# JaehaKim97/EDTR

Hardware: AMD Instinct MI355X
Metric: restored 512x512 images/sec @ 4 denoise steps (higher is better)
Workload: dtype bf16; 1 GPU; EDTR-det s4 (sd21): vae_encode + q_sample(t=200) + 4 x (ControlNet+UNet) + vae_decode, batch 8/GPU of 512x512; global_batch=8, image_size=512, denoise_steps=4, parallelism=batch-sharded x1, graphs=True, batches_in_flight=2, precision=fast

## Files before the change

edtr_amd/csrc/norm.hip:

```cpp
#include <stdlib.h>
#include "common.h"

namespace {

template <typename T>
struct IO16 {
    using in_t = uint16_t;
    using out_t = uint16_t;
    static __device__ __forceinline__ void load8(const in_t* p, float (&f)[8]) { unpack8<T>(ldg16(p), f); }
    static __device__ __forceinline__ void store8(out_t* p, int, const float (&f)[8]) { stg16(p, pack8<T>(f)); }
};
template <typename OT, int PARTS>
struct IOF32 {
    using in_t = float;
    using out_t = uint16_t;
    static __device__ __forceinline__ void load8(const in_t* p, float (&f)[8]) {
        const f32x4 a = *reinterpret_cast<const f32x4*>(p), b = *reinterpret_cast<const f32x4*>(p + 4);
#pragma unroll
        for (int j = 0; j < 4; ++j) { f[j] = a[j]; f[j + 4] = b[j]; }
    }
    static __device__ __forceinline__ void store8(out_t* p, int C, const float (&f)[8]) {
        const U4 hi = pack8<OT>(f);
        stg16(p, hi);
        if constexpr (PARTS >= 2) {
            float lo[8], back[8];
            unpack8<OT>(hi, back);
#pragma unroll
            for (int j = 0; j < 8; ++j) lo[j] = f[j] - back[j];
            stg16(p + C, pack8<OT>(lo));
        }
        if constexpr (PARTS == 3) stg16(p + 2 * C, hi);
    }
};
using IOF32S = IOF32<BF16, 3>;

template <typename F>
bool with_io(int dtype, F&& body) {
    switch (dtype) {
        case EDTR_BF16: body(IO16<BF16>{}); return true;
        case EDTR_F16: body(IO16<F16>{}); return true;
        case EDTR_F32_SPLIT: body(IOF32<BF16, 3>{}); return true;
        case EDTR_F32_H1: body(IOF32<F16, 1>{}); return true;
        case EDTR_F32_H2: body(IOF32<F16, 2>{}); return true;
        case EDTR_F32_H3: body(IOF32<F16, 3>{}); return true;
        default: return false;
    }
}

template <typename IO>
__global__ void gn_stats_kernel(const edtr_gn_params p, int CV, int R, int ppb) {
    using in_t = typename IO::in_t;
    extern __shared__ __attribute__((aligned(16))) char smem_raw[];
    float* red = reinterpret_cast<float*>(smem_raw);
    const int tid = threadIdx.x;
    const int b = blockIdx.y;
    const int C = p.C;
    const int cpg = C / p.groups;
    const int64_t pix0 = (int64_t)blockIdx.x * ppb;
    const int npix = (int)min((int64_t)ppb, (int64_t)p.HW - pix0);
    const in_t* xb = static_cast<const in_t*>(p.x) + ((int64_t)b * p.HW + pix0) * p.ldx;
    const int nslots = (CV + blockDim.x - 1) / blockDim.x;
    for (int slot = 0; slot < nslots; ++slot) {
        const int cv = R > 1 ? tid % CV : tid + slot * (int)blockDim.x;
        const int r = R > 1 ? tid / CV : 0;
        if (cv >= CV || r >= R) continue;
        float s[8], q[8];
#pragma unroll
        for (int j = 0; j < 8; ++j) { s[j] = 0.0f; q[j] = 0.0f; }
        const in_t* xp = xb + cv * 8;
        int pi = r;
        for (; pi + 3 * R < npix; pi += 4 * R) {
            float fv[4][8];
#pragma unroll
            for (int u = 0; u < 4; ++u) IO::load8(xp + (int64_t)(pi + u * R) * p.ldx, fv[u]);
#pragma unroll
            for (int u = 0; u < 4; ++u) {
#pragma unroll
                for (int j = 0; j < 8; ++j) { s[j] += fv[u][j]; q[j] += fv[u][j] * fv[u][j]; }
            }
        }
        for (; pi < npix; pi += R) {
            float f[8];
            IO::load8(xp + (int64_t)pi * p.ldx, f);
#pragma unroll
            for (int j = 0; j < 8; ++j) { s[j] += f[j]; q[j] += f[j] * f[j]; }
        }
#pragma unroll
        for (int j = 0; j < 8; ++j) {
            red[r * C + cv * 8 + j] = s[j];
            red[(R + r) * C + cv * 8 + j] = q[j];
        }
    }
    __syncthreads();
    for (int c = tid; c < C; c += blockDim.x) {
        float a = 0.0f, bq = 0.0f;
        for (int r = 0; r < R; ++r) { a += red[r * C + c]; bq += red[(R + r) * C + c]; }
        red[c] = a;
        red[R * C + c] = bq;
    }
    __syncthreads();
    if (tid < p.groups) {
        float a = 0.0f, bq = 0.0f;
        for (int c = tid * cpg; c < (tid + 1) * cpg; ++c) { a += red[c]; bq += red[R * C + c]; }
        double* dst = p.sums + ((int64_t)b * p.groups + tid) * 2;
        atomicAdd(dst, (double)a);
        atomicAdd(dst + 1, (double)bq);
    }
}

constexpr int GN_CC = 256;
__device__ int g_gn_apply_generic = 0;
__device__ __forceinline__ bool gn_apply_generic_only() { return g_gn_apply_generic != 0; }

template <typename IO>
__global__ void __launch_bounds__(256) gn_apply_kernel(const edtr_gn_params p, int ppb) {
    using in_t = typename IO::in_t;
    using out_t = typename IO::out_t;
    __shared__ __attribute__((aligned(16))) float sc[GN_CC];
    __shared__ __attribute__((aligned(16))) float sh[GN_CC];
    __shared__ double chan_s[GN_CC + 128], chan_q[GN_CC + 128];
    const int tid = threadIdx.x, b = blockIdx.z;
    const int c0 = blockIdx.y * GN_CC;
    const int cc = min(GN_CC, p.C - c0);
    const int cpg = p.C / p.groups;
    const double inv_cnt = 1.0 / ((double)p.HW * cpg);
    const int glo = (c0 / cpg) * cpg;
    if (p.partial) {
        const int ghi = min(p.C, ((c0 + cc + cpg - 1) / cpg) * cpg);
        for (int ch = glo + tid; ch < ghi; ch += 256) {
            const float* src = p.partial + ((int64_t)b * p.tiles_per_image * p.C + ch) * 2;
            double s = 0.0, q = 0.0;
            for (int t = 0; t < p.tiles_per_image; ++t) {
                const f32x2 v = *reinterpret_cast<const f32x2*>(src + (int64_t)t * p.C * 2);
                s += (double)v[0];
                q += (double)v[1];
            }
            chan_s[ch - glo] = s;
            chan_q[ch - glo] = q;
        }
        __syncthreads();
    }
    for (int c = tid; c < cc; c += 256) {
        double gsum[2];
        if (p.partial) {
            const int g0 = ((c0 + c) / cpg) * cpg - glo;
            double s = 0.0, q = 0.0;
            for (int j = 0; j < cpg; ++j) { s += chan_s[g0 + j]; q += chan_q[g0 + j]; }
            gsum[0] = s;
            gsum[1] = q;
        } else {
            const double* srcd = p.sums + ((int64_t)b * p.groups + (c0 + c) / cpg) * 2;
            gsum[0] = srcd[0];
            gsum[1] = srcd[1];
        }
        const double mean = gsum[0] * inv_cnt;
        double var = gsum[1] * inv_cnt - mean * mean;
        var = var < 0.0 ? 0.0 : var;
        const float rstd = __builtin_amdgcn_rsqf((float)var + p.eps);
        const float g = p.gamma[c0 + c] * rstd;
        sc[c] = g;
        sh[c] = p.beta[c0 + c] - (float)mean * g;
    }
    __syncthreads();
    const int ncv = cc >> 3;
    const int64_t pix0 = (int64_t)blockIdx.x * ppb;
    const int npix = (int)min((int64_t)ppb, (int64_t)p.HW - pix0);
    const in_t* xb = static_cast<const in_t*>(p.x) + ((int64_t)b * p.HW + pix0) * p.ldx + c0;
    out_t* yb = static_cast<out_t*>(p.y) + ((int64_t)b * p.HW + pix0) * p.ldy + c0;
    const int total = npix * ncv;
    if ((ncv & (ncv - 1)) == 0 && ncv <= 256 && !gn_apply_generic_only()) {
        const int sh_ = __builtin_ctz(ncv), cvf = tid & (ncv - 1), prow = tid >> sh_, pstep = 256 >> sh_;
        const f32x4 a0 = *reinterpret_cast<const f32x4*>(sc + cvf * 8), a1 = *reinterpret_cast<const f32x4*>(sc + cvf * 8 + 4);
        const f32x4 b0 = *reinterpret_cast<const f32x4*>(sh + cvf * 8), b1 = *reinterpret_cast<const f32x4*>(sh + cvf * 8 + 4);
        const in_t* xt = xb + cvf * 8;
        out_t* yt = yb + cvf * 8;
        for (int px0 = prow; px0 < npix; px0 += 4 * pstep) {
            float fv[4][8];
#pragma unroll
            for (int u = 0; u < 4; ++u)
                if (px0 + u * pstep < npix) IO::load8(xt + (int64_t)(px0 + u * pstep) * p.ldx, fv[u]);
#pragma unroll
            for (int u = 0; u < 4; ++u) {
                if (px0 + u * pstep >= npix) continue;
                float (&f)[8] = fv[u];
#pragma unroll
                for (int j = 0; j < 4; ++j) {
                    f[j] = f[j] * a0[j] + b0[j];
                    f[j + 4] = f[j + 4] * a1[j] + b1[j];
                }
                if (p.silu) {
#pragma unroll
                    for (int j = 0; j < 8; ++j) f[j] = silu_f(f[j]);
                }
                IO::store8(yt + (int64_t)(px0 + u * pstep) * p.ldy, p.C, f);
            }
        }
        return;
    }
    for (int i0 = tid; i0 < total; i0 += 4 * 256) {
        float fv[4][8];
        int pi[4], cv[4];
#pragma unroll
        for (int u = 0; u < 4; ++u) {
            const int i = i0 + u * 256;
            pi[u] = i / ncv;
            cv[u] = i - pi[u] * ncv;
            if (i < total) IO::load8(xb + (int64_t)pi[u] * p.ldx + cv[u] * 8, fv[u]);
        }
#pragma unroll
        for (int u = 0; u < 4; ++u) {
            if (i0 + u * 256 >= total) continue;
            float (&f)[8] = fv[u];
            const f32x4 a0 = *reinterpret_cast<const f32x4*>(sc + cv[u] * 8), a1 = *reinterpret_cast<const f32x4*>(sc + cv[u] * 8 + 4);
            const f32x4 b0 = *reinterpret_cast<const f32x4*>(sh + cv[u] * 8), b1 = *reinterpret_cast<const f32x4*>(sh + cv[u] * 8 + 4);
#pragma unroll
            for (int j = 0; j < 4; ++j) {
                f[j] = f[j] * a0[j] + b0[j];
                f[j + 4] = f[j + 4] * a1[j] + b1[j];
            }
            if (p.silu) {
#pragma unroll
                for (int j = 0; j < 8; ++j) f[j] = silu_f(f[j]);
            }
            IO::store8(yb + (int64_t)pi[u] * p.ldy + cv[u] * 8, p.C, f);
        }
    }
}

template <typename IO, bool PADDED>
__global__ void __launch_bounds__(256) layernorm_kernel(const typename IO::in_t* x, int64_t rows, int C, int c_valid, int ldx,
                                                       const float* gamma, const float* beta, float eps,
                                                       typename IO::out_t* y, int ldy) {
    const int lane = threadIdx.x & 63;
    const int64_t row = (int64_t)blockIdx.x * 4 + (threadIdx.x >> 6);
    if (row >= rows) return;
    const int CV = C >> 3;
    const float n_cols = (float)(PADDED ? c_valid : C);
    float f[4][8];
    float sum = 0.0f;
#pragma unroll
    for (int s = 0; s < 4; ++s) {
        const int cv = lane + 64 * s;
        if (cv < CV) {
            IO::load8(x + row * ldx + cv * 8, f[s]);
#pragma unroll
            for (int j = 0; j < 8; ++j) {
                if (PADDED && cv * 8 + j >= c_valid) f[s][j] = 0.0f;
                sum += f[s][j];
            }
        }
    }
    const float mean = wave_sum(sum) / n_cols;
    float sq = 0.0f;
#pragma unroll
    for (int s = 0; s < 4; ++s) {
        const int cv = lane + 64 * s;
        if (cv < CV) {
#pragma unroll
            for (int j = 0; j < 8; ++j) {
                const float d = f[s][j] - mean;
                if (!PADDED || cv * 8 + j < c_valid) sq += d * d;
            }
        }
    }
    const float rstd = rsqrtf(wave_sum(sq) / n_cols + eps);
#pragma unroll
    for (int s = 0; s < 4; ++s) {
        const int cv = lane + 64 * s;
        if (cv < CV) {
            float o[8];
#pragma unroll
            for (int j = 0; j < 8; ++j) {
                o[j] = (f[s][j] - mean) * rstd * gamma[cv * 8 + j] + beta[cv * 8 + j];
                if (PADDED && cv * 8 + j >= c_valid) o[j] = 0.0f;
            }
            IO::store8(y + row * ldy + cv * 8, C, o);
        }
    }
}

template <typename T>
__global__ void __launch_bounds__(256) softmax_rows_kernel(const float* s, int cols, int64_t ld_s, uint16_t* pout,
                                                          int64_t ld_p, int cols_pad) {
    __shared__ float red_m[4], red_l[4];
    const int tid = threadIdx.x, lane = tid & 63, wave = tid >> 6;
    const float* row = s + (int64_t)blockIdx.x * ld_s;
    uint16_t* orow = pout + (int64_t)blockIdx.x * ld_p;
    float m = -1e30f, l = 0.0f;
    for (int c = tid * 4; c < cols; c += 1024) {
        const f32x4 v = *reinterpret_cast<const f32x4*>(row + c);
        const float vm = fmaxf(fmaxf(v[0], v[1]), fmaxf(v[2], v[3]));
        const float mn = fmaxf(m, vm);
        l = l * __expf(m - mn) + __expf(v[0] - mn) + __expf(v[1] - mn) + __expf(v[2] - mn) + __expf(v[3] - mn);
        m = mn;
    }
    const float wm = wave_max(m);
    l = wave_sum(l * __expf(m - wm));
    if (lane == 0) { red_m[wave] = wm; red_l[wave] = l; }
    __syncthreads();
    const float gm = fmaxf(fmaxf(red_m[0], red_m[1]), fmaxf(red_m[2], red_m[3]));
    float gl = 0.0f;
#pragma unroll
    for (int w = 0; w < 4; ++w) gl += red_l[w] * __expf(red_m[w] - gm);
    const float inv = 1.0f / gl;
    for (int c = tid * 4; c < cols; c += 1024) {
        const f32x4 v = *reinterpret_cast<const f32x4*>(row + c);
        uint2 o;
        o.x = pack2<T>(__expf(v[0] - gm) * inv, __expf(v[1] - gm) * inv);
        o.y = pack2<T>(__expf(v[2] - gm) * inv, __expf(v[3] - gm) * inv);
        *reinterpret_cast<uint2*>(orow + c) = o;
    }
    for (int c = cols + tid * 4; c < cols_pad; c += 1024) *reinterpret_cast<uint2*>(orow + c) = make_uint2(0u, 0u);
}

int check_gn(const edtr_gn_params& p, bool apply) {
    if (!p.x || (!p.sums && !(apply && p.partial))) return EDTR_E_NULL;
    if (apply && (!p.y || !p.gamma || !p.beta)) return EDTR_E_NULL;
    if (p.dtype < EDTR_BF16 || p.dtype > EDTR_F32_H3) return EDTR_E_DTYPE;
    if (p.B <= 0 || p.HW <= 0 || p.C <= 0 || p.groups <= 0 || p.groups > 64) return EDTR_E_SHAPE;
    if (p.C % p.groups) return EDTR_E_SHAPE;
    if ((p.C & 7) || (p.ldx & 7) || (apply && (p.ldy & 7))) return EDTR_E_ALIGN;
    if (!aligned16(p.x) || (apply && !aligned16(p.y))) return EDTR_E_ALIGN;
    if (p.C > 8192) return EDTR_E_UNSUPPORTED;
    return EDTR_OK;
}

}

static int gn_pixels_per_block(int64_t HW, int B, int min_ppb, int max_chunks_per_image) {
    int64_t chunks = (1024 + B - 1) / B;
    if (chunks > max_chunks_per_image) chunks = max_chunks_per_image;
    int64_t ppb = (HW + chunks - 1) / chunks;
    if (ppb < min_ppb) ppb = min_ppb;
    return (int)ppb;
}

extern "C" int edtr_gn_stats(const edtr_gn_params* pp, edtr_stream_t stream) {
    if (!pp) return EDTR_E_NULL;
    const edtr_gn_params& p = *pp;
    if (int e = check_gn(p, false)) return e;
    hipStream_t s = static_cast<hipStream_t>(stream);
    if (!p.sums_zeroed) {
        hipError_t e = hipMemsetAsync(p.sums, 0, sizeof(double) * 2 * p.groups * p.B, s);
        if (e != hipSuccess) return (int)e;
    }
    const int CV = p.C >> 3;
    int R = CV >= 256 ? 1 : 256 / CV;
    if (R < 1) R = 1;
    int threads = CV >= 256 ? 256 : CV * R;
    threads = ((threads + 63) / 64) * 64;
    if (threads < 64) threads = 64;
    const int ppb = gn_pixels_per_block(p.HW, p.B, 16, 64);
    dim3 grid((unsigned)((p.HW + ppb - 1) / ppb), p.B);
    const size_t lds = sizeof(float) * 2 * R * p.C;
    if (p.dtype == EDTR_BF16)
        hipLaunchKernelGGL(gn_stats_kernel<IO16<BF16>>, grid, dim3(threads), lds, s, p, CV, R, ppb);
    else if (p.dtype == EDTR_F16)
        hipLaunchKernelGGL(gn_stats_kernel<IO16<F16>>, grid, dim3(threads), lds, s, p, CV, R, ppb);
    else
        hipLaunchKernelGGL(gn_stats_kernel<IOF32S>, grid, dim3(threads), lds, s, p, CV, R, ppb);
    EDTR_LAUNCH_CHECK();
    return EDTR_OK;
}

extern "C" int edtr_gn_apply(const edtr_gn_params* pp, edtr_stream_t stream) {
    if (!pp) return EDTR_E_NULL;
    const edtr_gn_params& p = *pp;
    if (int e = check_gn(p, true)) return e;
    if (p.partial) {
        const int cpg = p.C / p.groups;
        if (p.tiles_per_image <= 0 || p.tiles_per_image > 64 || ((int64_t)p.tiles_per_image * 128 != p.HW && (int64_t)p.tiles_per_image * 64 != p.HW))
            return EDTR_E_SHAPE;
        if (cpg > 64) return EDTR_E_UNSUPPORTED;
    }
    hipStream_t s = static_cast<hipStream_t>(stream);
    static int generic = -1;
    if (generic < 0) {
        const char* e = getenv("EDTR_GN_APPLY_GENERIC");
        generic = (e && e[0] == '1') ? 1 : 0;
        if (generic) (void)hipMemcpyToSymbol(HIP_SYMBOL(g_gn_apply_generic), &generic, sizeof(int));
    }
    const int nchunk_c = (p.C + GN_CC - 1) / GN_CC;
    int64_t want = (2048 + (int64_t)p.B * nchunk_c - 1) / ((int64_t)p.B * nchunk_c);
    if (want < 1) want = 1;
    int64_t ppb = (p.HW + want - 1) / want;
    if (ppb < 8) ppb = 8;
    if (ppb > 256) ppb = 256;
    dim3 grid((unsigned)((p.HW + ppb - 1) / ppb), nchunk_c, p.B);
    with_io(p.dtype, [&](auto io) {
        hipLaunchKernelGGL(gn_apply_kernel<decltype(io)>, grid, dim3(256), 0, s, p, (int)ppb);
    });
    EDTR_LAUNCH_CHECK();
    return EDTR_OK;
}

namespace {
__global__ void gn_pool_kernel(double* sums, const float* weights, const float* counts, int T, int BG) {
    const int i = blockIdx.x * blockDim.x + threadIdx.x;
    if (i >= BG) return;
    double mean = 0.0, var = 0.0;
    for (int t = 0; t < T; ++t) {
        const double* s = sums + ((int64_t)t * BG + i) * 2;
        const double c = (double)counts[t];
        const double m = s[0] / c;
        double v = s[1] / c - m * m;
        v = v < 0.0 ? 0.0 : v;
        mean += (double)weights[t] * m;
        var += (double)weights[t] * v;
    }
    for (int t = 0; t < T; ++t) {
        double* s = sums + ((int64_t)t * BG + i) * 2;
        const double c = (double)counts[t];
        s[0] = mean * c;
        s[1] = (var + mean * mean) * c;
    }
}
}

extern "C" int edtr_gn_pool(double* sums, const float* weights, const float* counts, int T, int BG, edtr_stream_t stream) {
    if (!sums || !weights || !counts) return EDTR_E_NULL;
    if (T <= 0 || BG <= 0) return EDTR_E_SHAPE;
    hipLaunchKernelGGL(gn_pool_kernel, dim3((BG + 255) / 256), dim3(256), 0, static_cast<hipStream_t>(stream), sums, weights,
                       counts, T, BG);
    EDTR_LAUNCH_CHECK();
    return EDTR_OK;
}

extern "C" int edtr_layernorm(int dtype, const void* x, int64_t rows, int C, int c_valid, int ldx, const float* gamma,
                              const float* beta, float eps, void* y, int ldy, edtr_stream_t stream) {
    if (!x || !y || !gamma || !beta) return EDTR_E_NULL;
    if (dtype < EDTR_BF16 || dtype > EDTR_F32_H3) return EDTR_E_DTYPE;
    if (rows <= 0 || C <= 0 || c_valid < 0 || c_valid > C) return EDTR_E_SHAPE;
    if (C > 2048) return EDTR_E_UNSUPPORTED;
    if ((C & 7) || (ldx & 7) || (ldy & 7) || !aligned16(x) || !aligned16(y)) return EDTR_E_ALIGN;
    if (c_valid == 0) c_valid = C;
    hipStream_t s = static_cast<hipStream_t>(stream);
    dim3 grid((unsigned)((rows + 3) / 4));
    const uint16_t* xp = static_cast<const uint16_t*>(x);
    uint16_t* yp = static_cast<uint16_t*>(y);
    if (dtype >= EDTR_F32_SPLIT) {
        if (c_valid != C) return EDTR_E_UNSUPPORTED;
        with_io(dtype, [&](auto io) {
            using IO = decltype(io);
            if constexpr (sizeof(typename IO::in_t) == 4)
                hipLaunchKernelGGL((layernorm_kernel<IO, false>), grid, dim3(256), 0, s, static_cast<const float*>(x), rows, C, C, ldx, gamma, beta, eps, yp, ldy);
        });
    } else if (dtype == EDTR_BF16) {
        if (c_valid == C) hipLaunchKernelGGL((layernorm_kernel<IO16<BF16>, false>), grid, dim3(256), 0, s, xp, rows, C, C, ldx, gamma, beta, eps, yp, ldy);
        else hipLaunchKernelGGL((layernorm_kernel<IO16<BF16>, true>), grid, dim3(256), 0, s, xp, rows, C, c_valid, ldx, gamma, beta, eps, yp, ldy);
    } else {
        if (c_valid == C) hipLaunchKernelGGL((layernorm_kernel<IO16<F16>, false>), grid, dim3(256), 0, s, xp, rows, C, C, ldx, gamma, beta, eps, yp, ldy);
        else hipLaunchKernelGGL((layernorm_kernel<IO16<F16>, true>), grid, dim3(256), 0, s, xp, rows, C, c_valid, ldx, gamma, beta, eps, yp, ldy);
    }
    EDTR_LAUNCH_CHECK();
    return EDTR_OK;
}

extern "C" int edtr_softmax_rows(int dtype, const float* sc, int64_t rows, int cols, int64_t ld_s, void* pr,
                                 int64_t ld_p, int cols_pad, edtr_stream_t stream) {
    if (!sc || !pr) return EDTR_E_NULL;
    if (dtype != EDTR_BF16 && dtype != EDTR_F16) return EDTR_E_DTYPE;
    if (rows <= 0 || cols <= 0 || rows > 0x7fffffffLL) return EDTR_E_SHAPE;
    if ((cols & 3) || (ld_s & 3) || (ld_p & 3) || (cols_pad & 3) || !aligned16(sc) || (reinterpret_cast<uintptr_t>(pr) & 7))
        return EDTR_E_ALIGN;
    if (cols_pad < cols) cols_pad = cols;
    if (cols_pad > ld_p) return EDTR_E_SHAPE;
    hipStream_t s = static_cast<hipStream_t>(stream);
    if (dtype == EDTR_BF16)
        hipLaunchKernelGGL(softmax_rows_kernel<BF16>, dim3((unsigned)rows), dim3(256), 0, s, sc, cols, ld_s,
                           static_cast<uint16_t*>(pr), ld_p, cols_pad);
    else
        hipLaunchKernelGGL(softmax_rows_kernel<F16>, dim3((unsigned)rows), dim3(256), 0, s, sc, cols, ld_s,
                           static_cast<uint16_t*>(pr), ld_p, cols_pad);
    EDTR_LAUNCH_CHECK();
    return EDTR_OK;
}
```

Before: 123.9 images/s.

## Add persistent prefetching GroupNorm apply and multi-row-per-wave LayerNorm kernels

GroupNorm apply gains a persistent-grid variant that walks units of rows with a capped workgroup count. Each unit's raw loads are issued before the scale/shift reduction, and the next unit is double-buffered while the current one is normalized. LayerNorm gets a specialised kernel for C in {320, 640, 1280} that packs several rows per wavefront, uses lane-group shuffle reductions and stages gamma/beta in shared memory. Both changes target latency and occupancy on memory-bound norm passes, at the cost of more registers, code size and new env-controlled paths.

Result: no change. 124.3 images/s (median of 2 runs) (+0.3%).

```diff
diff --git a/edtr_amd/csrc/norm.hip b/edtr_amd/csrc/norm.hip
--- a/edtr_amd/csrc/norm.hip
+++ b/edtr_amd/csrc/norm.hip
@@ -7,6 +7,10 @@
 struct IO16 {
     using in_t = uint16_t;
     using out_t = uint16_t;
+    using raw_t = U4;
+    static __device__ __forceinline__ raw_t load_raw(const in_t* p) { return ldg16(p); }
+    static __device__ __forceinline__ raw_t zero_raw() { return zero16(); }
+    static __device__ __forceinline__ void cvt(const raw_t& r, float (&f)[8]) { unpack8<T>(r, f); }
     static __device__ __forceinline__ void load8(const in_t* p, float (&f)[8]) { unpack8<T>(ldg16(p), f); }
     static __device__ __forceinline__ void store8(out_t* p, int, const float (&f)[8]) { stg16(p, pack8<T>(f)); }
 };
@@ -14,11 +18,16 @@
 struct IOF32 {
     using in_t = float;
     using out_t = uint16_t;
-    static __device__ __forceinline__ void load8(const in_t* p, float (&f)[8]) {
-        const f32x4 a = *reinterpret_cast<const f32x4*>(p), b = *reinterpret_cast<const f32x4*>(p + 4);
-#pragma unroll
-        for (int j = 0; j < 4; ++j) { f[j] = a[j]; f[j + 4] = b[j]; }
-    }
+    struct raw_t { f32x4 a, b; };
+    static __device__ __forceinline__ raw_t load_raw(const in_t* p) {
+        return raw_t{*reinterpret_cast<const f32x4*>(p), *reinterpret_cast<const f32x4*>(p + 4)};
+    }
+    static __device__ __forceinline__ raw_t zero_raw() { return raw_t{f32x4{0.0f, 0.0f, 0.0f, 0.0f}, f32x4{0.0f, 0.0f, 0.0f, 0.0f}}; }
+    static __device__ __forceinline__ void cvt(const raw_t& r, float (&f)[8]) {
+#pragma unroll
+        for (int j = 0; j < 4; ++j) { f[j] = r.a[j]; f[j + 4] = r.b[j]; }
+    }
+    static __device__ __forceinline__ void load8(const in_t* p, float (&f)[8]) { cvt(load_raw(p), f); }
     static __device__ __forceinline__ void store8(out_t* p, int C, const float (&f)[8]) {
         const U4 hi = pack8<OT>(f);
         stg16(p, hi);
@@ -112,16 +121,9 @@
 __device__ int g_gn_apply_generic = 0;
 __device__ __forceinline__ bool gn_apply_generic_only() { return g_gn_apply_generic != 0; }
 
-template <typename IO>
-__global__ void __launch_bounds__(256) gn_apply_kernel(const edtr_gn_params p, int ppb) {
-    using in_t = typename IO::in_t;
-    using out_t = typename IO::out_t;
-    __shared__ __attribute__((aligned(16))) float sc[GN_CC];
-    __shared__ __attribute__((aligned(16))) float sh[GN_CC];
-    __shared__ double chan_s[GN_CC + 128], chan_q[GN_CC + 128];
-    const int tid = threadIdx.x, b = blockIdx.z;
-    const int c0 = blockIdx.y * GN_CC;
-    const int cc = min(GN_CC, p.C - c0);
+__device__ __forceinline__ void gn_scale_shift(const edtr_gn_params& p, int b, int c0, int cc, float* sc, float* sh, double* chan_s,
+                                               double* chan_q) {
+    const int tid = threadIdx.x;
     const int cpg = p.C / p.groups;
     const double inv_cnt = 1.0 / ((double)p.HW * cpg);
     const int glo = (c0 / cpg) * cpg;
@@ -162,67 +164,132 @@
         sh[c] = p.beta[c0 + c] - (float)mean * g;
     }
     __syncthreads();
+}
+
+template <typename IO>
+__device__ __forceinline__ void gn_norm_store8(float (&f)[8], const f32x4& a0, const f32x4& a1, const f32x4& b0, const f32x4& b1, int silu,
+                                               typename IO::out_t* dst, int C) {
+#pragma unroll
+    for (int j = 0; j < 4; ++j) {
+        f[j] = f[j] * a0[j] + b0[j];
+        f[j + 4] = f[j + 4] * a1[j] + b1[j];
+    }
+#ifndef EDTR_DIAG_NO_SILU
+    if (silu) {
+#pragma unroll
+        for (int j = 0; j < 8; ++j) f[j] = silu_f(f[j]);
+    }
+#endif
+    IO::store8(dst, C, f);
+}
+
+template <typename IO, int U>
+__global__ void __launch_bounds__(256) gn_apply_kernel(const edtr_gn_params p, int ppb) {
+    using in_t = typename IO::in_t;
+    using out_t = typename IO::out_t;
+    using raw_t = typename IO::raw_t;
+    __shared__ __attribute__((aligned(16))) float sc[GN_CC];
+    __shared__ __attribute__((aligned(16))) float sh[GN_CC];
+    __shared__ double chan_s[GN_CC + 128], chan_q[GN_CC + 128];
+    const int tid = threadIdx.x, b = blockIdx.z;
+    const int c0 = blockIdx.y * GN_CC;
+    const int cc = min(GN_CC, p.C - c0);
     const int ncv = cc >> 3;
-    const int64_t pix0 = (int64_t)blockIdx.x * ppb;
-    const int npix = (int)min((int64_t)ppb, (int64_t)p.HW - pix0);
-    const in_t* xb = static_cast<const in_t*>(p.x) + ((int64_t)b * p.HW + pix0) * p.ldx + c0;
-    out_t* yb = static_cast<out_t*>(p.y) + ((int64_t)b * p.HW + pix0) * p.ldy + c0;
-    const int total = npix * ncv;
-    if ((ncv & (ncv - 1)) == 0 && ncv <= 256 && !gn_apply_generic_only()) {
+    const in_t* xi = static_cast<const in_t*>(p.x) + (int64_t)b * p.HW * p.ldx + c0;
+    out_t* yi = static_cast<out_t*>(p.y) + (int64_t)b * p.HW * p.ldy + c0;
+    if ((ncv & (ncv - 1)) == 0 && !gn_apply_generic_only()) {
         const int sh_ = __builtin_ctz(ncv), cvf = tid & (ncv - 1), prow = tid >> sh_, pstep = 256 >> sh_;
-        const f32x4 a0 = *reinterpret_cast<const f32x4*>(sc + cvf * 8), a1 = *reinterpret_cast<const f32x4*>(sc + cvf * 8 + 4);
-        const f32x4 b0 = *reinterpret_cast<const f32x4*>(sh + cvf * 8), b1 = *reinterpret_cast<const f32x4*>(sh + cvf * 8 + 4);
-        const in_t* xt = xb + cvf * 8;
-        out_t* yt = yb + cvf * 8;
-        for (int px0 = prow; px0 < npix; px0 += 4 * pstep) {
+        if constexpr (U == 0) {
+            gn_scale_shift(p, b, c0, cc, sc, sh, chan_s, chan_q);
+            const f32x4 a0 = *reinterpret_cast<const f32x4*>(sc + cvf * 8), a1 = *reinterpret_cast<const f32x4*>(sc + cvf * 8 + 4);
+            const f32x4 b0 = *reinterpret_cast<const f32x4*>(sh + cvf * 8), b1 = *reinterpret_cast<const f32x4*>(sh + cvf * 8 + 4);
+            const int64_t pix0 = (int64_t)blockIdx.x * ppb;
+            const int npix = (int)min((int64_t)ppb, (int64_t)p.HW - pix0);
+            const in_t* xt = xi + pix0 * p.ldx + cvf * 8;
+            out_t* yt = yi + pix0 * p.ldy + cvf * 8;
+            for (int px0 = prow; px0 < npix; px0 += 4 * pstep) {
+                float fv[4][8];
+#pragma unroll
+                for (int u = 0; u < 4; ++u)
+                    if (px0 + u * pstep < npix) IO::load8(xt + (int64_t)(px0 + u * pstep) * p.ldx, fv[u]);
+#pragma unroll
+                for (int u = 0; u < 4; ++u) {
+                    if (px0 + u * pstep >= npix) continue;
+                    gn_norm_store8<IO>(fv[u], a0, a1, b0, b1, p.silu, yt + (int64_t)(px0 + u * pstep) * p.ldy, p.C);
+                }
+            }
+        } else {
+            const int urows = U * pstep, nunits = (p.HW + urows - 1) / urows;
+            const in_t* xt = xi + cvf * 8;
+            out_t* yt = yi + cvf * 8;
+            auto load_unit = [&](int u, raw_t (&r)[U]) {
+                const int px = u * urows + prow;
+                if ((u + 1) * urows <= p.HW) {
+    #pragma unroll
+                    for (int k = 0; k < U; ++k) r[k] = IO::load_raw(xt + (int64_t)(px + k * pstep) * p.ldx);
+                } else {
+    #pragma unroll
+                    for (int k = 0; k < U; ++k) r[k] = px + k * pstep < p.HW ? IO::load_raw(xt + (int64_t)(px + k * pstep) * p.ldx) : IO::zero_raw();
+                }
+            };
+            raw_t cur[U], nxt[U];
+            int u = blockIdx.x;
+            if (u < nunits) load_unit(u, cur);
+            gn_scale_shift(p, b, c0, cc, sc, sh, chan_s, chan_q);
+            if (u >= nunits) return;
+            const f32x4 a0 = *reinterpret_cast<const f32x4*>(sc + cvf * 8), a1 = *reinterpret_cast<const f32x4*>(sc + cvf * 8 + 4);
+            const f32x4 b0 = *reinterpret_cast<const f32x4*>(sh + cvf * 8), b1 = *reinterpret_cast<const f32x4*>(sh + cvf * 8 + 4);
+            for (;;) {
+                const int un = u + (int)gridDim.x;
+                const bool more = un < nunits;
+                if (more) load_unit(un, nxt);
+                const int px = u * urows + prow;
+                if ((u + 1) * urows <= p.HW) {
+    #pragma unroll
+                    for (int k = 0; k < U; ++k) {
+                        float f[8];
+                        IO::cvt(cur[k], f);
+                        gn_norm_store8<IO>(f, a0, a1, b0, b1, p.silu, yt + (int64_t)(px + k * pstep) * p.ldy, p.C);
+                    }
+                } else {
+    #pragma unroll
+                    for (int k = 0; k < U; ++k) {
+                        if (px + k * pstep >= p.HW) continue;
+                        float f[8];
+                        IO::cvt(cur[k], f);
+                        gn_norm_store8<IO>(f, a0, a1, b0, b1, p.silu, yt + (int64_t)(px + k * pstep) * p.ldy, p.C);
+                    }
+                }
+                if (!more) break;
+                for (int k = 0; k < U; ++k) cur[k] = nxt[k];
+                u = un;
+            }
+        }
+        return;
+    }
+    gn_scale_shift(p, b, c0, cc, sc, sh, chan_s, chan_q);
+    for (int64_t pix0 = (int64_t)blockIdx.x * ppb; pix0 < p.HW; pix0 += (int64_t)gridDim.x * ppb) {
+        const int npix = (int)min((int64_t)ppb, (int64_t)p.HW - pix0);
+        const in_t* xb = xi + pix0 * p.ldx;
+        out_t* yb = yi + pix0 * p.ldy;
+        const int total = npix * ncv;
+        for (int i0 = tid; i0 < total; i0 += 4 * 256) {
             float fv[4][8];
-#pragma unroll
-            for (int u = 0; u < 4; ++u)
-                if (px0 + u * pstep < npix) IO::load8(xt + (int64_t)(px0 + u * pstep) * p.ldx, fv[u]);
+            int pi[4], cv[4];
 #pragma unroll
             for (int u = 0; u < 4; ++u) {
-                if (px0 + u * pstep >= npix) continue;
-                float (&f)[8] = fv[u];
-#pragma unroll
-                for (int j = 0; j < 4; ++j) {
-                    f[j] = f[j] * a0[j] + b0[j];
-                    f[j + 4] = f[j + 4] * a1[j] + b1[j];
-                }
-                if (p.silu) {
-#pragma unroll
-                    for (int j = 0; j < 8; ++j) f[j] = silu_f(f[j]);
-                }
-                IO::store8(yt + (int64_t)(px0 + u * pstep) * p.ldy, p.C, f);
-            }
-        }
-        return;
-    }
-    for (int i0 = tid; i0 < total; i0 += 4 * 256) {
-        float fv[4][8];
-        int pi[4], cv[4];
-#pragma unroll
-        for (int u = 0; u < 4; ++u) {
-            const int i = i0 + u * 256;
-            pi[u] = i / ncv;
-            cv[u] = i - pi[u] * ncv;
-            if (i < total) IO::load8(xb + (int64_t)pi[u] * p.ldx + cv[u] * 8, fv[u]);
-        }
-#pragma unroll
-        for (int u = 0; u < 4; ++u) {
-            if (i0 + u * 256 >= total) continue;
-            float (&f)[8] = fv[u];
-            const f32x4 a0 = *reinterpret_cast<const f32x4*>(sc + cv[u] * 8), a1 = *reinterpret_cast<const f32x4*>(sc + cv[u] * 8 + 4);
-            const f32x4 b0 = *reinterpret_cast<const f32x4*>(sh + cv[u] * 8), b1 = *reinterpret_cast<const f32x4*>(sh + cv[u] * 8 + 4);
-#pragma unroll
-            for (int j = 0; j < 4; ++j) {
-                f[j] = f[j] * a0[j] + b0[j];
-                f[j + 4] = f[j + 4] * a1[j] + b1[j];
-            }
-            if (p.silu) {
-#pragma unroll
-                for (int j = 0; j < 8; ++j) f[j] = silu_f(f[j]);
-            }
-            IO::store8(yb + (int64_t)pi[u] * p.ldy + cv[u] * 8, p.C, f);
+                const int i = i0 + u * 256;
+                pi[u] = i / ncv;
+                cv[u] = i - pi[u] * ncv;
+                if (i < total) IO::load8(xb + (int64_t)pi[u] * p.ldx + cv[u] * 8, fv[u]);
+            }
+#pragma unroll
+            for (int u = 0; u < 4; ++u) {
+                if (i0 + u * 256 >= total) continue;
+                const f32x4 a0 = *reinterpret_cast<const f32x4*>(sc + cv[u] * 8), a1 = *reinterpret_cast<const f32x4*>(sc + cv[u] * 8 + 4);
+                const f32x4 b0 = *reinterpret_cast<const f32x4*>(sh + cv[u] * 8), b1 = *reinterpret_cast<const f32x4*>(sh + cv[u] * 8 + 4);
+                gn_norm_store8<IO>(fv[u], a0, a1, b0, b1, p.silu, yb + (int64_t)pi[u] * p.ldy + cv[u] * 8, p.C);
+            }
         }
     }
 }
@@ -277,6 +344,82 @@
             IO::store8(y + row * ldy + cv * 8, C, o);
         }
     }
+}
+
+template <int LG>
+__device__ __forceinline__ float lane_group_sum(float v) {
+#pragma unroll
+    for (int o = LG / 2; o > 0; o >>= 1) v += __shfl_xor(v, o, 64);
+    return v;
+}
+
+template <typename IO, int LG>
+__global__ void __launch_bounds__(256) layernorm_rows_kernel(const typename IO::in_t* x, int64_t rows, int ldx, const float* gamma,
+                                                            const float* beta, float eps, typename IO::out_t* y, int ldy) {
+    using raw_t = typename IO::raw_t;
+    constexpr int RPW = 64 / LG, C = 40 * LG;
+    const int lane = threadIdx.x & 63, gl = lane & (LG - 1), rsub = lane / LG;
+    const int64_t nwaves = (int64_t)gridDim.x * 4;
+    __shared__ __attribute__((aligned(16))) float gs[C], bs[C];
+    for (int c = threadIdx.x * 4; c < C; c += 256 * 4) {
+        *reinterpret_cast<f32x4*>(gs + c) = *reinterpret_cast<const f32x4*>(gamma + c);
+        *reinterpret_cast<f32x4*>(bs + c) = *reinterpret_cast<const f32x4*>(beta + c);
+    }
+    __syncthreads();
+    for (int64_t r0 = ((int64_t)blockIdx.x * 4 + (threadIdx.x >> 6)) * RPW; r0 < rows; r0 += nwaves * RPW) {
+        const int64_t row = r0 + rsub;
+        const bool live = row < rows;
+        raw_t raw[5];
+#pragma unroll
+        for (int s = 0; s < 5; ++s) raw[s] = live ? IO::load_raw(x + row * ldx + (gl + LG * s) * 8) : IO::zero_raw();
+        float f[5][8];
+        float sum = 0.0f;
+#pragma unroll
+        for (int s = 0; s < 5; ++s) {
+            IO::cvt(raw[s], f[s]);
+#pragma unroll
+            for (int j = 0; j < 8; ++j) sum += f[s][j];
+        }
+        const float mean = lane_group_sum<LG>(sum) / (float)C;
+        float sq = 0.0f;
+#pragma unroll
+        for (int s = 0; s < 5; ++s) {
+#pragma unroll
+            for (int j = 0; j < 8; ++j) {
+                const float d = f[s][j] - mean;
+                sq += d * d;
+            }
+        }
+        const float rstd = rsqrtf(lane_group_sum<LG>(sq) / (float)C + eps);
+        if (!live) continue;
+#pragma unroll
+        for (int s = 0; s < 5; ++s) {
+            const int c = (gl + LG * s) * 8;
+            const f32x4 g0 = *reinterpret_cast<const f32x4*>(gs + c), g1 = *reinterpret_cast<const f32x4*>(gs + c + 4);
+            const f32x4 t0 = *reinterpret_cast<const f32x4*>(bs + c), t1 = *reinterpret_cast<const f32x4*>(bs + c + 4);
+            float o[8];
+#pragma unroll
+            for (int j = 0; j < 4; ++j) {
+                o[j] = (f[s][j] - mean) * rstd * g0[j] + t0[j];
+                o[j + 4] = (f[s][j + 4] - mean) * rstd * g1[j] + t1[j];
+            }
+            IO::store8(y + row * ldy + (gl + LG * s) * 8, C, o);
+        }
+    }
+}
+
+template <typename IO>
+bool launch_layernorm_rows(const typename IO::in_t* x, int64_t rows, int C, int ldx, const float* gamma, const float* beta, float eps,
+                           typename IO::out_t* y, int ldy, hipStream_t s) {
+    if (C != 320 && C != 640 && C != 1280) return false;
+    if (!aligned16(gamma) || !aligned16(beta)) return false;
+    const int rpb = 4 * 64 / (C / 40);
+    int64_t nb = (rows + rpb - 1) / rpb;
+    if (nb > 1024) nb = 1024;
+    if (C == 320) hipLaunchKernelGGL((layernorm_rows_kernel<IO, 8>), dim3((unsigned)nb), dim3(256), 0, s, x, rows, ldx, gamma, beta, eps, y, ldy);
+    else if (C == 640) hipLaunchKernelGGL((layernorm_rows_kernel<IO, 16>), dim3((unsigned)nb), dim3(256), 0, s, x, rows, ldx, gamma, beta, eps, y, ldy);
+    else hipLaunchKernelGGL((layernorm_rows_kernel<IO, 32>), dim3((unsigned)nb), dim3(256), 0, s, x, rows, ldx, gamma, beta, eps, y, ldy);
+    return true;
 }
 
 template <typename T>
@@ -380,15 +523,35 @@
         generic = (e && e[0] == '1') ? 1 : 0;
         if (generic) (void)hipMemcpyToSymbol(HIP_SYMBOL(g_gn_apply_generic), &generic, sizeof(int));
     }
+    static int wgs = 0;
+    if (wgs <= 0) {
+        const char* e = getenv("EDTR_GN_APPLY_WGS");
+        wgs = e ? atoi(e) : 0;
+        if (wgs < 256 || wgs > 65536) wgs = 2048;
+    }
     const int nchunk_c = (p.C + GN_CC - 1) / GN_CC;
-    int64_t want = (2048 + (int64_t)p.B * nchunk_c - 1) / ((int64_t)p.B * nchunk_c);
+    const int64_t per_x = (int64_t)p.B * nchunk_c;
+    int64_t want = (2048 + per_x - 1) / per_x;
     if (want < 1) want = 1;
     int64_t ppb = (p.HW + want - 1) / want;
     if (ppb < 8) ppb = 8;
     if (ppb > 256) ppb = 256;
-    dim3 grid((unsigned)((p.HW + ppb - 1) / ppb), nchunk_c, p.B);
+    int64_t gx = (p.HW + ppb - 1) / ppb;
+    const int ncv0 = (p.C < GN_CC ? p.C : GN_CC) >> 3;
+    bool walk = false;
+    if ((ncv0 & (ncv0 - 1)) == 0 && !generic) {
+        const int urows = 4 * (256 / ncv0);
+        const int64_t nunits = (p.HW + urows - 1) / urows;
+        if (nunits * per_x >= 4 * (int64_t)wgs) {
+            walk = true;
+            gx = (wgs + per_x - 1) / per_x;
+        }
+    }
+    dim3 grid((unsigned)gx, nchunk_c, p.B);
     with_io(p.dtype, [&](auto io) {
-        hipLaunchKernelGGL(gn_apply_kernel<decltype(io)>, grid, dim3(256), 0, s, p, (int)ppb);
+        using IO = decltype(io);
+        if (walk) hipLaunchKernelGGL((gn_apply_kernel<IO, 4>), grid, dim3(256), 0, s, p, (int)ppb);
+        else hipLaunchKernelGGL((gn_apply_kernel<IO, 0>), grid, dim3(256), 0, s, p, (int)ppb);
     });
     EDTR_LAUNCH_CHECK();
     return EDTR_OK;
@@ -436,6 +599,11 @@
     if (c_valid == 0) c_valid = C;
     hipStream_t s = static_cast<hipStream_t>(stream);
     dim3 grid((unsigned)((rows + 3) / 4));
+    static int one_row_per_wave = -1;
+    if (one_row_per_wave < 0) {
+        const char* e = getenv("EDTR_LN_ONE_ROW_PER_WAVE");
+        one_row_per_wave = (e && e[0] == '1') ? 1 : 0;
+    }
     const uint16_t* xp = static_cast<const uint16_t*>(x);
     uint16_t* yp = static_cast<uint16_t*>(y);
     if (dtype >= EDTR_F32_SPLIT) {
@@ -446,10 +614,12 @@
                 hipLaunchKernelGGL((layernorm_kernel<IO, false>), grid, dim3(256), 0, s, static_cast<const float*>(x), rows, C, C, ldx, gamma, beta, eps, yp, ldy);
         });
     } else if (dtype == EDTR_BF16) {
-        if (c_valid == C) hipLaunchKernelGGL((layernorm_kernel<IO16<BF16>, false>), grid, dim3(256), 0, s, xp, rows, C, C, ldx, gamma, beta, eps, yp, ldy);
+        if (c_valid == C && !one_row_per_wave && launch_layernorm_rows<IO16<BF16>>(xp, rows, C, ldx, gamma, beta, eps, yp, ldy, s)) {}
+        else if (c_valid == C) hipLaunchKernelGGL((layernorm_kernel<IO16<BF16>, false>), grid, dim3(256), 0, s, xp, rows, C, C, ldx, gamma, beta, eps, yp, ldy);
         else hipLaunchKernelGGL((layernorm_kernel<IO16<BF16>, true>), grid, dim3(256), 0, s, xp, rows, C, c_valid, ldx, gamma, beta, eps, yp, ldy);
     } else {
-        if (c_valid == C) hipLaunchKernelGGL((layernorm_kernel<IO16<F16>, false>), grid, dim3(256), 0, s, xp, rows, C, C, ldx, gamma, beta, eps, yp, ldy);
+        if (c_valid == C && !one_row_per_wave && launch_layernorm_rows<IO16<F16>>(xp, rows, C, ldx, gamma, beta, eps, yp, ldy, s)) {}
+        else if (c_valid == C) hipLaunchKernelGGL((layernorm_kernel<IO16<F16>, false>), grid, dim3(256), 0, s, xp, rows, C, C, ldx, gamma, beta, eps, yp, ldy);
         else hipLaunchKernelGGL((layernorm_kernel<IO16<F16>, true>), grid, dim3(256), 0, s, xp, rows, C, c_valid, ldx, gamma, beta, eps, yp, ldy);
     }
     EDTR_LAUNCH_CHECK();
```
